# VinAIResearch/GeoFormer

Hardware: AMD Instinct MI355X
Metric: scenes/sec forward (ScanNetV2 ~150k pts) (higher is better)
Workload: dtype f32

## Files before the change

geoformer_amd/_lib.py:

```python
from __future__ import annotations

import ctypes
import os
from ctypes import c_char_p, c_float, c_int, c_longlong, c_size_t, c_uint, c_void_p

from ._build import LIB_PATH

LIB_PATH = os.environ.get("GF_LIB_PATH", LIB_PATH)

_lib = None


class GeoFormerHipError(RuntimeError):
    pass


def _declare(lib):
    P, I, F = c_void_p, c_int, c_float
    sig = {
        "gf_abi_version": (I, []),
        "gf_last_error": (c_char_p, []),
        "gf_index_words": (c_size_t, [I, I, I, I]),
        "gf_index_scratch_bytes": (c_size_t, [c_size_t]),
        "gf_index_build": (I, [P, I, P, I, I, I, I, P, P, P, P, P]),
# ... 15 lines not shown
        "gf_conv_dual_supported": (I, [I, I, I, I, I]),
        "gf_rules_flat_words": (c_size_t, [I, I]),
        "gf_rules_flat_steps": (I, [P, P, I, I, I, I, P, P]),
        "gf_conv_fwd_flat": (I, [P, P, P, P, P, P, I, I, I, I, I, I, P, P, P, P, P, P, P, P]),
        "gf_conv_fwd_dual": (I, [P, P, P, P, P, I, I, I, I, I, I, P, P, P, P, P, P, P, P]),
        "gf_dev_conv_fwd_timed": (I, [P, P, P, P, P, I, I, I, I, I, I, P, P, P, P, P, P, P, P, P]),
        "gf_dev_conv_knobs_g16": (I, [I, I, I, I]),
        "gf_dev_conv_chunks": (I, [I]),
        "gf_dev_conv_g16p_wpb": (I, [I]),
        "gf_dev_conv_knobs": (I, [I, I, I, I, I]),
        "gf_dev_conv_knob_flat": (I, [I, I]),
        "gf_dev_conv_knob_lw": (I, [I, I]),
        "gf_dev_conv_plan": (I, [P, P, P, P, P, P, I, I, I, I, I, I, P, P, P, P, P, P, P, P]),
        "gf_resblock_fwd": (I, [P, P, P, P, P, P, P, I, I, I, I, I, P, P, P, P, P, P, P, P]),
        "gf_conv_wgrad": (I, [P, P, P, I, I, I, I, I, P, P]),
        "gf_conv_wgrad_masked": (I, [P, P, P, P, I, I, I, I, I, P, P]),
        "gf_conv_wgrad_masked_acc": (I, [P, P, P, P, I, I, I, I, I, P, P]),
        "gf_lsap": (I, [P, I, I, P, P, P, P, P, P]),
        "gf_pair_losses_sums_floats": (c_size_t, [I]),
        "gf_pair_losses_fwd": (I, [P, P, P, I, I, I, P, P, P, P]),
        "gf_pair_losses_bwd": (I, [P, P, P, P, I, I, I, P, P, P, P]),
        "gf_unet_ws_bytes": (c_size_t, [P, I, I, I, I, I]),
        "gf_dev_unet_probe": (I, [I]),
        "gf_dev_host_wait_ns": (ctypes.c_ulonglong, [I]),
        "gf_dev_unet_probe_read": (I, [I, P, P]),
        "gf_dev_unet_probe_read2": (I, [I, P, P, P]),
        "gf_dev_conv_kernel_events": (I, [P, P]),
        "gf_dev_conv_kernel_events_taken": (I, []),
        "gf_dev_op_kernel_events": (I, [I, P, P]),
        "gf_dev_op_kernel_events_taken": (I, [I]),
        "gf_dev_event_create": (P, []),
        "gf_dev_event_destroy": (I, [P]),
        "gf_dev_event_elapsed_us": (I, [P, P, P]),
        "gf_unet_fwd": (I, [P, P, P, I, I, I, I, I, P, c_size_t, P, P, P, P]),
        "gf_unet_fwd_phased": (I, [P, P, P, I, I, I, I, I, P, c_size_t, P, P, P, P, P, I, P, P]),
        "gf_unet_fwd_ahead": (I, [P, P, P, I, I, I, I, I, P, c_size_t, P, P, P, P, P, I]),
        "gf_voxelize_fp": (I, [P, P, I, I, I, I, P, P]),
        "gf_voxelize_bp": (I, [P, P, I, I, I, I, P, P]),
        "gf_gather_points": (I, [P, P, I, I, I, I, P, P]),
        "gf_gather_points_grad": (I, [P, P, I, I, I, I, P, P]),
        "gf_group_points": (I, [P, P, I, I, I, I, I, P, P]),
        "gf_group_points_grad": (I, [P, P, I, I, I, I, I, P, P]),
        "gf_ball_query": (I, [P, P, I, I, I, F, I, P, P]),
        "gf_fps_scratch_bytes": (c_size_t, [I]),
        "gf_furthest_point_sampling": (I, [P, I, I, I, P, P, P]),
        "gf_furthest_point_sampling_resume": (I, [P, I, I, I, I, P, P, P]),
        "gf_knn_scratch_bytes": (c_size_t, [I]),
        "gf_knn_radius": (I, [P, I, I, F, I, P, P, P, P, P]),
        "gf_knn_error_flag": (P, [P, I]),
        "gf_geodesic_bfs": (I, [P, P, P, I, I, P, I, F, I, P, P, P, P]),
        "gf_geodesic_bfs_cfg": (I, [P, P, P, I, I, P, I, F, I, P, P, P, c_size_t, I, P]),
        "gf_geodesic_bfs_queue_words": (c_size_t, [I]),
        "gf_dev_cross_attn_bf3": (I, [I]),
        "gf_dev_bfs_qcap_max": (I, [I]),
        "gf_mask_head": (I, [P, P, P, P, P, P, P, P, P, I, I, I, P, P]),
        "gf_mask_head_packed": (I, [P, P, P, P, P, P, P, P, P, I, I, I, I, P, P]),
        "gf_mask_head_episodes": (I, [P, P, P, P, P, P, P, P, P, I, I, I, I, I, P, P, P]),
        "gf_mask_head_split_bytes": (c_size_t, [I]),
        "gf_mask_head_bwd": (I, [P, P, P, P, P, P, P, P, P, I, I, I, I, P, P, P, P]),
        "gf_mask_head_bwd_episodes": (I, [P, P, P, P, P, P, P, P, P, I, I, I, I, I, P, P, P, P]),
        "gf_mask_head_bwd_scratch_floats": (c_size_t, [I, I]),
        "gf_softmax_dim1_fwd": (I, [P, I, I, I, F, P, P]),
        "gf_softmax_dim1_bwd": (I, [P, P, I, I, I, F, P, P]),
        "gf_pointwise_mlp": (I, [P, I, I, P, P, P, P, P, P, P]),
        "gf_pointwise_mlp_rows": (I, [P, P, I, I, P, P, P, P, P, P, P]),
        "gf_group_mlp_max": (I, [P, I, I, I, I, P, P, P, P, P, P, P]),
        "gf_ball_query_centres": (I, [P, P, I, I, I, F, I, P, P, P]),
        "gf_sa_group_mlp_max": (I, [P, P, P, I, I, I, I, F, I, I, I, I, P, P, P, P, P, P, P, P, P, I, P]),
        "gf_ball_query_grid": (I, [P, I, P, P, I, F, I, P, I, P, P, P]),
        "gf_point_grid_build": (I, [P, I, F, P, P]),
        "gf_decoder_token_state_bytes": (c_size_t, [I, I]),
        "gf_decoder_token_stage": (I, [P, P, P, I, I, I, I, I, P, P, P, P, P, P]),
        "gf_mask_intersections_scratch_bytes": (c_size_t, [I, I]),
        "gf_mask_intersections": (I, [P, I, I, P, P, P]),
        "gf_proposal_stats_batched": (I, [P, I, I, P, P, c_longlong, I, F, F, I, I, P, P, P, P, P]),
        "gf_proposal_select_batched": (I, [P, P, P, I, I, P, P, P, P, P]),
        "gf_proposal_scatter_batched": (I, [P, I, I, P, P, I, I, P, F, P, P]),
        "gf_mask_intersections_batched": (I, [P, I, c_longlong, c_longlong, P, P, P]),
        "gf_matrix_nms_batched": (I, [P, I, P, I, F, F, P, P, P]),
        "gf_label_map_batched": (I, [P, I, c_longlong, I, F, P, P, P, P, P, P, P, P, P]),
        "gf_instance_overlaps_scratch_bytes": (c_size_t, [I, I]),
        "gf_instance_overlaps": (I, [P, I, I, P, I, P, P, I, I, P, P, P, P, P, P]),
        "gf_voxelize_idx_scratch_bytes": (c_size_t, [I]),
        "gf_voxelize_idx_count": (I, [P, I, I, I, P, P, P, P]),
        "gf_voxelize_idx_fill": (I, [P, I, I, I, P, P, I, I, P, P, P]),
        "gf_host_legacy_choice": (I, [P, P, c_longlong, c_longlong, P]),
        "gf_host_legacy_prefetch": (I, [P, I, c_longlong]),
        "gf_host_draw_sample": (I, [P, P, c_longlong, c_longlong, P, c_longlong, P, P, P, P, I, P, P, P]),
        "gf_fg_scratch_bytes": (c_size_t, [I]),
        "gf_fg_select": (I, [P, I, I, I, I, P, P, P, P, I, P, P, P, P, P, P, P, P, P]),
        "gf_host_wait_word": (I, [P, I, c_longlong]),
        "gf_proposal_stats": (I, [P, P, P, I, I, I, F, F, I, I, P, P, P, P, P]),
        "gf_proposal_stats_fs": (I, [P, P, I, I, F, F, I, F, P, P, P, P]),
        "gf_proposal_scatter": (I, [P, P, I, I, P, F, I, P, P]),
        "gf_relpos_prepare": (I, [P, P, I, I, I, P, P, P]),
        "gf_proposal_select": (I, [P, P, P, I, P, P, P, P, P]),
        "gf_backbone_transformer_scratch_bytes": (c_size_t, [I]),
        "gf_backbone_transformer_num_params": (I, [I]),
        "gf_backbone_transformer": (I, [P, P, P, I, I, I, I, P, P, P, P]),
        "gf_decoder_pre_train_save_bytes": (c_size_t, [I, I]),
        "gf_decoder_pre_train_work_bytes": (c_size_t, [I, I]),
        "gf_decoder_pre_grad_floats": (c_longlong, []),
        "gf_decoder_pre_train_fwd": (I, [P, P, I, I, P, F, c_uint, I, P, P, P, P]),
        "gf_decoder_pre_train_bwd": (I, [P, P, P, P, P, I, I, P, F, c_uint, I, P, P, P, P, P, P]),
        "gf_decoder_post_train_save_bytes": (c_size_t, [I, I, I]),
        "gf_decoder_post_train_work_bytes": (c_size_t, [I, I, I]),
# ... 150 lines not shown
```

geoformer_amd/csrc/decoder_attn.hip:

```cpp
#include <stdlib.h>

#include "common.h"

#define DA_WAVES 16
#define DA_D 64

__device__ __forceinline__ float da_row_max(float v) {
    v = fmaxf(v, __int_as_float(__builtin_amdgcn_update_dpp(0, __float_as_int(v), 0xB1, 0xF, 0xF, true)));
    v = fmaxf(v, __int_as_float(__builtin_amdgcn_update_dpp(0, __float_as_int(v), 0x4E, 0xF, 0xF, true)));
    v = fmaxf(v, __int_as_float(__builtin_amdgcn_update_dpp(0, __float_as_int(v), 0x141, 0xF, 0xF, true)));
    v = fmaxf(v, __int_as_float(__builtin_amdgcn_update_dpp(0, __float_as_int(v), 0x140, 0xF, 0xF, true)));
    return v;
}
__device__ __forceinline__ float da_row_sum(float v) {
    v += __int_as_float(__builtin_amdgcn_update_dpp(0, __float_as_int(v), 0xB1, 0xF, 0xF, true));
    v += __int_as_float(__builtin_amdgcn_update_dpp(0, __float_as_int(v), 0x4E, 0xF, 0xF, true));
    v += __int_as_float(__builtin_amdgcn_update_dpp(0, __float_as_int(v), 0x141, 0xF, 0xF, true));
    v += __int_as_float(__builtin_amdgcn_update_dpp(0, __float_as_int(v), 0x140, 0xF, 0xF, true));
    return v;
}

template <int WAVES>
__global__ __launch_bounds__(WAVES * 64) void k_decoder_cross_attn(
    const float* __restrict__ geo_ctx, const float* __restrict__ max_geo, const float* __restrict__ qloc,
    const float* __restrict__ cloc, const float* __restrict__ lo, const float* __restrict__ hi,
    const float* __restrict__ gaussB, const float* __restrict__ Q1, const float* __restrict__ K1,
    const float* __restrict__ Kv, const float4* __restrict__ Wpack, int nq, int nc, float* __restrict__ out,
    float* __restrict__ stat_m, float* __restrict__ stat_l) {
    __shared__ float4 sW[3 * 16 * 64];
    __shared__ float4 sQ1[16];
    __shared__ float4 sB[3][2][4];
    __shared__ float sRed[3][WAVES][DA_D];
    const int qi = blockIdx.x, b = blockIdx.y;
    const int tid = threadIdx.x, lane = tid & 63, w = tid >> 6, g = lane >> 4, j = lane & 15;
    for (int t = tid; t < 3 * 16 * 64; t += WAVES * 64) sW[t] = Wpack[t];
    if (tid < 16) sQ1[tid] = *reinterpret_cast<const float4*>(Q1 + ((size_t)b * nq + qi) * DA_D + tid * 4);
    if (tid >= 64 && tid < 64 + 24) {
        const int e = tid - 64, axis = e >> 3, half = (e >> 2) & 1, gg = e & 3;
        sB[axis][half][gg] = *reinterpret_cast<const float4*>(gaussB + axis * 32 + half * 16 + 4 * gg);
    }
    geo_ctx += ((size_t)b * nq + qi) * nc;
    cloc += (size_t)b * nc * 3;
    K1 += (size_t)b * nc * DA_D;
    Kv += (size_t)b * nc * DA_D;
    const float mg = max_geo[(size_t)b * nq + qi];
    const float qx = qloc[((size_t)b * nq + qi) * 3 + 0], qy = qloc[((size_t)b * nq + qi) * 3 + 1],
                qz = qloc[((size_t)b * nq + qi) * 3 + 2];
    const float lx = lo[b * 3 + 0], ly = lo[b * 3 + 1], lz = lo[b * 3 + 2];
    const float sx = hi[b * 3 + 0] - lx, sy = hi[b * 3 + 1] - ly, sz = hi[b * 3 + 2] - lz;
    float sm[4][4], sl[4][4], sa[4][4];
#pragma unroll
    for (int rb = 0; rb < 4; rb++)
#pragma unroll
        for (int r = 0; r < 4; r++) {
            sm[rb][r] = -3.0e38f;
// ... 78 lines not shown
                    const float corr = __expf(sm[rb][r] - mn), p = __expf(x - mn);
                    sl[rb][r] = sl[rb][r] * corr + p;
                    sa[rb][r] = sa[rb][r] * corr + p * val;
                    sm[rb][r] = mn;
                }
            }
            __builtin_amdgcn_sched_barrier(0);
        }
    }
#pragma unroll
    for (int rb = 0; rb < 4; rb++)
#pragma unroll
        for (int r = 0; r < 4; r++) {
            const float m = da_row_max(sm[rb][r]);
            if (j == 0) sRed[0][w][rb * 16 + 4 * g + r] = m;
        }
    __syncthreads();
    if (tid < DA_D) {
        float m = sRed[0][0][tid];
#pragma unroll
        for (int u = 1; u < WAVES; u++) m = fmaxf(m, sRed[0][u][tid]);
        sRed[0][0][tid] = m;
    }
    __syncthreads();
#pragma unroll
    for (int rb = 0; rb < 4; rb++)
#pragma unroll
        for (int r = 0; r < 4; r++) {
            const int c = rb * 16 + 4 * g + r;
            const float f = __expf(sm[rb][r] - sRed[0][0][c]);
            const float l = da_row_sum(sl[rb][r] * f), a = da_row_sum(sa[rb][r] * f);
            if (j == 0) {
                sRed[1][w][c] = l;
                sRed[2][w][c] = a;
            }
        }
    __syncthreads();
    if (tid < DA_D) {
        float L = 0.f, A = 0.f;
#pragma unroll
        for (int u = 0; u < WAVES; u++) {
            L += sRed[1][u][tid];
            A += sRed[2][u][tid];
        }
        out[((size_t)b * nq + qi) * DA_D + tid] = A / L;
        if (stat_m) {
            stat_m[((size_t)b * nq + qi) * DA_D + tid] = sRed[0][0][tid];
            stat_l[((size_t)b * nq + qi) * DA_D + tid] = L;
        }
    }
}

#define DA_WPACK_F32 (3 * 16 * 64 * 4)
#define DA_WPACK_BF3_U4 (3 * 4 * 2 * 3 * 64)
__device__ __forceinline__ void da_split3(float x, unsigned& h, unsigned& m, unsigned& l) {
    h = __float_as_uint(x) & 0xffff0000u;
    const float r1 = x - __uint_as_float(h);
    m = __float_as_uint(r1) & 0xffff0000u;
    l = __float_as_uint(r1 - __uint_as_float(m));
}
typedef __bf16 da_bf16x8 __attribute__((ext_vector_type(8)));
typedef unsigned da_u32x4 __attribute__((ext_vector_type(4)));
struct DaPieces {
    da_u32x4 p[2][3];
};
__device__ __forceinline__ void da_split_pack(const float (&x)[4][4], DaPieces& P) {
#pragma unroll
    for (int h = 0; h < 2; h++) {
        unsigned pc[3][8];
#pragma unroll
        for (int e = 0; e < 8; e++) da_split3(x[2 * h + (e >> 2)][e & 3], pc[0][e], pc[1][e], pc[2][e]);
#pragma unroll
        for (int piece = 0; piece < 3; piece++)
#pragma unroll
            for (int i = 0; i < 4; i++)
                P.p[h][piece][i] = __builtin_amdgcn_perm(pc[piece][2 * i + 1], pc[piece][2 * i], 0x07060302u);
    }
}

#ifndef DA_BF3_WAVES
#define DA_BF3_WAVES 16
#endif
template <int NT>
__device__ __forceinline__ void da_gemm_bf3_n(const uint4* __restrict__ sW3, int m, int rb, int lane, const DaPieces (&X)[NT],
                                              f32x4 (&acc)[NT]) {
#pragma unroll
    for (int h = 0; h < 2; h++) {
        const uint4* w = sW3 + (size_t)(((m * 4 + rb) * 2 + h) * 3) * 64 + lane;
        const da_bf16x8 ah = __builtin_bit_cast(da_bf16x8, w[0]), am = __builtin_bit_cast(da_bf16x8, w[64]),
                        al = __builtin_bit_cast(da_bf16x8, w[128]);
#pragma unroll
        for (int u = 0; u < NT; u++) acc[u] = __builtin_amdgcn_mfma_f32_16x16x32_bf16(al, __builtin_bit_cast(da_bf16x8, X[u].p[h][0]), acc[u], 0, 0, 0);
#pragma unroll
        for (int u = 0; u < NT; u++) acc[u] = __builtin_amdgcn_mfma_f32_16x16x32_bf16(ah, __builtin_bit_cast(da_bf16x8, X[u].p[h][2]), acc[u], 0, 0, 0);
#pragma unroll
        for (int u = 0; u < NT; u++) acc[u] = __builtin_amdgcn_mfma_f32_16x16x32_bf16(am, __builtin_bit_cast(da_bf16x8, X[u].p[h][1]), acc[u], 0, 0, 0);
#pragma unroll
        for (int u = 0; u < NT; u++) acc[u] = __builtin_amdgcn_mfma_f32_16x16x32_bf16(am, __builtin_bit_cast(da_bf16x8, X[u].p[h][0]), acc[u], 0, 0, 0);
#pragma unroll
        for (int u = 0; u < NT; u++) acc[u] = __builtin_amdgcn_mfma_f32_16x16x32_bf16(ah, __builtin_bit_cast(da_bf16x8, X[u].p[h][1]), acc[u], 0, 0, 0);
#pragma unroll
        for (int u = 0; u < NT; u++) acc[u] = __builtin_amdgcn_mfma_f32_16x16x32_bf16(ah, __builtin_bit_cast(da_bf16x8, X[u].p[h][0]), acc[u], 0, 0, 0);
    }
}

template <int WAVES, int NT>
__global__ __launch_bounds__(WAVES * 64) void k_decoder_cross_attn_bf3(
    const float* __restrict__ geo_ctx, const float* __restrict__ max_geo, const float* __restrict__ qloc,
    const float* __restrict__ cloc, const float* __restrict__ lo, const float* __restrict__ hi,
    const float* __restrict__ gaussB, const float* __restrict__ Q1, const float* __restrict__ K1,
    const float* __restrict__ Kv, const uint4* __restrict__ Wp3, int nq, int nc, float* __restrict__ out,
    float* __restrict__ stat_m, float* __restrict__ stat_l) {
    extern __shared__ __attribute__((aligned(16))) unsigned char da_smem[];
    uint4* sW3 = reinterpret_cast<uint4*>(da_smem);
    __shared__ float4 sQ1[16];
    __shared__ float4 sB[3][2][4];
    __shared__ float sRed[3][WAVES][DA_D];
    const int qi = blockIdx.x, b = blockIdx.y;
    const int tid = threadIdx.x, lane = tid & 63, w = tid >> 6, g = lane >> 4, j = lane & 15;
    for (int t = tid; t < DA_WPACK_BF3_U4; t += WAVES * 64) sW3[t] = Wp3[t];
    if (tid < 16) sQ1[tid] = *reinterpret_cast<const float4*>(Q1 + ((size_t)b * nq + qi) * DA_D + tid * 4);
    if (tid >= 64 && tid < 64 + 24) {
        const int e = tid - 64, axis = e >> 3, half = (e >> 2) & 1, gg = e & 3;
        sB[axis][half][gg] = *reinterpret_cast<const float4*>(gaussB + axis * 32 + half * 16 + 4 * gg);
    }
    geo_ctx += ((size_t)b * nq + qi) * nc;
    cloc += (size_t)b * nc * 3;
    K1 += (size_t)b * nc * DA_D;
    Kv += (size_t)b * nc * DA_D;
    const float mg = max_geo[(size_t)b * nq + qi];
    const float qx = qloc[((size_t)b * nq + qi) * 3 + 0], qy = qloc[((size_t)b * nq + qi) * 3 + 1],
                qz = qloc[((size_t)b * nq + qi) * 3 + 2];
    const float lx = lo[b * 3 + 0], ly = lo[b * 3 + 1], lz = lo[b * 3 + 2];
    const float ix = 1.0f / (hi[b * 3 + 0] - lx), iy = 1.0f / (hi[b * 3 + 1] - ly), iz = 1.0f / (hi[b * 3 + 2] - lz);
    constexpr float kScale2 = 0.125f * 1.44269504088896341f;
    float sm[4][4], sl[4][4], sa[4][4];
#pragma unroll
    for (int rb = 0; rb < 4; rb++)
#pragma unroll
        for (int r = 0; r < 4; r++) {
            sm[rb][r] = -3.0e38f;
            sl[rb][r] = 0.f;
            sa[rb][r] = 0.f;
        }
    __syncthreads();

    const int ntiles = (nc + 15) >> 4;
    for (int t0 = w * NT; t0 < ntiles; t0 += WAVES * NT) {
        bool valid[NT];
        int cc[NT];
        DaPieces RP[NT];
#pragma unroll
        for (int u = 0; u < NT; u++) {
            const int ctx = (t0 + u) * 16 + j;
            valid[u] = ctx < nc;
            cc[u] = valid[u] ? ctx : nc - 1;
            const float gd = geo_ctx[cc[u]];
            float g0 = gd, g1 = gd, g2 = gd;
            if (gd < 0.f) {
                g0 = mg + fabsf(qx - cloc[cc[u] * 3 + 0]);
                g1 = mg + fabsf(qy - cloc[cc[u] * 3 + 1]);
                g2 = mg + fabsf(qz - cloc[cc[u] * 3 + 2]);
            }
            const float t0f = (g0 - lx) * ix, t1f = (g1 - ly) * iy, t2f = (g2 - lz) * iz;
            float R[4][4];
#pragma unroll
            for (int half = 0; half < 2; half++) {
                const float4 b0 = sB[0][half][g], b1 = sB[1][half][g], b2v = sB[2][half][g];
                const float p[4] = {fmaf(t2f, b2v.x, fmaf(t1f, b1.x, t0f * b0.x)), fmaf(t2f, b2v.y, fmaf(t1f, b1.y, t0f * b0.y)),
                                    fmaf(t2f, b2v.z, fmaf(t1f, b1.z, t0f * b0.z)), fmaf(t2f, b2v.w, fmaf(t1f, b1.w, t0f * b0.w))};
#pragma unroll
                for (int e = 0; e < 4; e++) {
                    R[half][e] = __builtin_amdgcn_sinf(p[e]);
                    R[2 + half][e] = __builtin_amdgcn_cosf(p[e]);
                }
            }
            da_split_pack(R, RP[u]);
        }
        float H[NT][4][4];
        f32x4 V[NT][4];
#pragma unroll
        for (int rb = 0; rb < 4; rb++) {
            f32x4 acc[NT], vv[NT];
#pragma unroll
            for (int u = 0; u < NT; u++) {
                acc[u] = (f32x4){0.f, 0.f, 0.f, 0.f};
                vv[u] = (f32x4){0.f, 0.f, 0.f, 0.f};
            }
            da_gemm_bf3_n<NT>(sW3, 0, rb, lane, RP, acc);
            const float4 q1 = sQ1[rb * 4 + g];
#pragma unroll
            for (int u = 0; u < NT; u++) {
                const float4 k1 = *reinterpret_cast<const float4*>(K1 + (size_t)cc[u] * DA_D + rb * 16 + 4 * g);
                H[u][rb][0] = fmaxf(acc[u][0] + q1.x - k1.x, 0.f);
                H[u][rb][1] = fmaxf(acc[u][1] + q1.y - k1.y, 0.f);
                H[u][rb][2] = fmaxf(acc[u][2] + q1.z - k1.z, 0.f);
                H[u][rb][3] = fmaxf(acc[u][3] + q1.w - k1.w, 0.f);
            }
            da_gemm_bf3_n<NT>(sW3, 2, rb, lane, RP, vv);
#pragma unroll
            for (int u = 0; u < NT; u++) V[u][rb] = vv[u];
            __builtin_amdgcn_sched_barrier(0);
        }
        DaPieces HP[NT];
#pragma unroll
        for (int u = 0; u < NT; u++) da_split_pack(H[u], HP[u]);
#pragma unroll
        for (int rb = 0; rb < 4; rb++) {
            f32x4 s[NT];
#pragma unroll
            for (int u = 0; u < NT; u++) s[u] = (f32x4){0.f, 0.f, 0.f, 0.f};
            da_gemm_bf3_n<NT>(sW3, 1, rb, lane, HP, s);
#pragma unroll
            for (int u = 0; u < NT; u++) {
                const float4 kv = *reinterpret_cast<const float4*>(Kv + (size_t)cc[u] * DA_D + rb * 16 + 4 * g);
                const float kvv[4] = {kv.x, kv.y, kv.z, kv.w};
                if (valid[u]) {
#pragma unroll
                    for (int r = 0; r < 4; r++) {
                        const float x = s[u][r] * kScale2;
                        const float val = V[u][rb][r] + kvv[r];
                        const float mn = fmaxf(sm[rb][r], x);
                        const float corr = __builtin_amdgcn_exp2f(sm[rb][r] - mn), p = __builtin_amdgcn_exp2f(x - mn);
                        sl[rb][r] = sl[rb][r] * corr + p;
                        sa[rb][r] = sa[rb][r] * corr + p * val;
                        sm[rb][r] = mn;
                    }
                }
            }
            __builtin_amdgcn_sched_barrier(0);
        }
    }
#pragma unroll
    for (int rb = 0; rb < 4; rb++)
#pragma unroll
        for (int r = 0; r < 4; r++) {
            const float m = da_row_max(sm[rb][r]);
            if (j == 0) sRed[0][w][rb * 16 + 4 * g + r] = m;
        }
    __syncthreads();
    if (tid < DA_D) {
        float m = sRed[0][0][tid];
#pragma unroll
        for (int u = 1; u < WAVES; u++) m = fmaxf(m, sRed[0][u][tid]);
        sRed[0][0][tid] = m;
    }
    __syncthreads();
#pragma unroll
    for (int rb = 0; rb < 4; rb++)
#pragma unroll
        for (int r = 0; r < 4; r++) {
            const int c = rb * 16 + 4 * g + r;
            const float f = __builtin_amdgcn_exp2f(sm[rb][r] - sRed[0][0][c]);
            const float l = da_row_sum(sl[rb][r] * f), a = da_row_sum(sa[rb][r] * f);
            if (j == 0) {
                sRed[1][w][c] = l;
                sRed[2][w][c] = a;
            }
        }
    __syncthreads();
    if (tid < DA_D) {
        float L = 0.f, A = 0.f;
#pragma unroll
        for (int u = 0; u < WAVES; u++) {
            L += sRed[1][u][tid];
            A += sRed[2][u][tid];
        }
        out[((size_t)b * nq + qi) * DA_D + tid] = A / L;
        if (stat_m) {
            stat_m[((size_t)b * nq + qi) * DA_D + tid] = sRed[0][0][tid] * 0.69314718055994531f;
            stat_l[((size_t)b * nq + qi) * DA_D + tid] = L;
        }
    }
}

extern "C" size_t gf_decoder_wpack_floats(void) { return (size_t)DA_WPACK_F32 + (size_t)DA_WPACK_BF3_U4 * 4; }

__global__ void k_decoder_pack(const float* __restrict__ W1, const float* __restrict__ W2, const float* __restrict__ Wv,
                               float* __restrict__ Wp) {
    const int t = blockIdx.x * blockDim.x + threadIdx.x;
    if (t >= 3 * 16 * 64 * 4) return;
    const int s = t & 3, lane = (t >> 2) & 63, kb = (t >> 8) & 3, rb = (t >> 10) & 3, m = t >> 12;
    const float* W = m == 0 ? W1 : (m == 1 ? W2 : Wv);
    Wp[t] = W[(rb * 16 + (lane & 15)) * DA_D + kb * 16 + 4 * (lane >> 4) + s];
}

__global__ void k_decoder_pack_bf3(const float* __restrict__ W1, const float* __restrict__ W2, const float* __restrict__ Wv,
                                   uint4* __restrict__ Wp3) {
    const int t = blockIdx.x * blockDim.x + threadIdx.x;
    if (t >= 3 * 4 * 2 * 64) return;
    const int lane = t & 63, h = (t >> 6) & 1, rb = (t >> 7) & 3, m = t >> 9;
    const float* W = m == 0 ? W1 : (m == 1 ? W2 : Wv);
    unsigned pc[3][8];
    for (int e = 0; e < 8; e++) {
        const int kb = 2 * h + (e >> 2), sidx = e & 3;
        da_split3(W[(rb * 16 + (lane & 15)) * DA_D + kb * 16 + 4 * (lane >> 4) + sidx], pc[0][e], pc[1][e], pc[2][e]);
    }
    for (int piece = 0; piece < 3; piece++) {
        uint4 v;
        v.x = (pc[piece][1] & 0xffff0000u) | (pc[piece][0] >> 16);
        v.y = (pc[piece][3] & 0xffff0000u) | (pc[piece][2] >> 16);
        v.z = (pc[piece][5] & 0xffff0000u) | (pc[piece][4] >> 16);
        v.w = (pc[piece][7] & 0xffff0000u) | (pc[piece][6] >> 16);
        Wp3[((size_t)(((m * 4 + rb) * 2 + h) * 3 + piece)) * 64 + lane] = v;
    }
}

extern "C" int gf_decoder_pack_weights(const float* W1, const float* W2, const float* Wv, float* Wpack, void* stream) {
    hipLaunchKernelGGL(k_decoder_pack, dim3(48), dim3(256), 0, (hipStream_t)stream, W1, W2, Wv, Wpack);
    hipLaunchKernelGGL(k_decoder_pack_bf3, dim3(6), dim3(256), 0, (hipStream_t)stream, W1, W2, Wv,
                       reinterpret_cast<uint4*>(Wpack + DA_WPACK_F32));
    GF_CHECK_LAUNCH("gf_decoder_pack_weights");
    return GF_OK;
}

static int g_da_bf3 = -1;
extern "C" int gf_dev_cross_attn_bf3(int on) {
    g_da_bf3 = on < 0 ? -1 : (on != 0);
    return GF_OK;
}

extern "C" int gf_decoder_cross_attn_cfg(const float* geo_ctx, const float* max_geo, const float* qloc, const float* cloc,
                                         const float* lo, const float* hi, const float* gaussB, const float* Q1,
                                         const float* K1, const float* Kv, const float* Wpack, const float* b2, int B,
                                         int nq, int nc, int d, float* out, float* stat_m, float* stat_l, int wg_waves,
                                         void* stream) {
    GF_CHECK_ARG(d == DA_D, "gf_decoder_cross_attn: implemented for dec_dim = 64 (got %d)", d);
    GF_CHECK_ARG(B >= 0 && nq >= 0 && nc >= 1, "gf_decoder_cross_attn: bad sizes");
    GF_CHECK_ARG((stat_m == nullptr) == (stat_l == nullptr), "gf_decoder_cross_attn: stat_m and stat_l come together");
    GF_CHECK_ARG(wg_waves == 16 || wg_waves == 8, "gf_decoder_cross_attn_cfg: %d waves per workgroup (16 or 8)", wg_waves);
    if (B == 0 || nq == 0) return GF_OK;
    (void)b2;
    if (wg_waves == 16 && g_da_bf3 != 0) {
        const size_t lds = (size_t)DA_WPACK_BF3_U4 * sizeof(uint4);
        gf_allow_lds((const void*)k_decoder_cross_attn_bf3<DA_BF3_WAVES, 1>, (int)lds);
        GF_LAUNCH_OP(GF_OP_CROSS_ATTN, (k_decoder_cross_attn_bf3<DA_BF3_WAVES, 1>), dim3(nq, B), dim3(DA_BF3_WAVES * 64), lds,
                     (hipStream_t)stream, geo_ctx, max_geo, qloc, cloc, lo, hi, gaussB, Q1, K1, Kv,
                     reinterpret_cast<const uint4*>(Wpack + DA_WPACK_F32), nq, nc, out, stat_m, stat_l);
        GF_CHECK_LAUNCH("gf_decoder_cross_attn");
        return GF_OK;
    }
    if (wg_waves == 16)
        GF_LAUNCH_OP(GF_OP_CROSS_ATTN, k_decoder_cross_attn<16>, dim3(nq, B), dim3(16 * 64), 0, (hipStream_t)stream, geo_ctx,
                     max_geo, qloc, cloc, lo, hi, gaussB, Q1, K1, Kv, reinterpret_cast<const float4*>(Wpack), nq, nc, out,
                     stat_m, stat_l);
    else
        GF_LAUNCH_OP(GF_OP_CROSS_ATTN, k_decoder_cross_attn<8>, dim3(nq, B), dim3(8 * 64), 0, (hipStream_t)stream, geo_ctx,
                     max_geo, qloc, cloc, lo, hi, gaussB, Q1, K1, Kv, reinterpret_cast<const float4*>(Wpack), nq, nc, out,
                     stat_m, stat_l);
    GF_CHECK_LAUNCH("gf_decoder_cross_attn");
    return GF_OK;
}

extern "C" int gf_decoder_cross_attn(const float* geo_ctx, const float* max_geo, const float* qloc, const float* cloc,
                                     const float* lo, const float* hi, const float* gaussB, const float* Q1,
                                     const float* K1, const float* Kv, const float* Wpack, const float* b2, int B,
                                     int nq, int nc, int d, float* out, float* stat_m, float* stat_l, void* stream) {
    return gf_decoder_cross_attn_cfg(geo_ctx, max_geo, qloc, cloc, lo, hi, gaussB, Q1, K1, Kv, Wpack, b2, B, nq, nc, d, out,
                                     stat_m, stat_l, 16, stream);
}


#define DAB_TS 68

__global__ void k_decoder_pack_w2t(const float* __restrict__ W2, float* __restrict__ Wp) {
    const int t = blockIdx.x * blockDim.x + threadIdx.x;
    if (t >= 16 * 64 * 4) return;
    const int s = t & 3, lane = (t >> 2) & 63, kb = (t >> 8) & 3, cb = (t >> 10) & 3;
    Wp[t] = W2[(kb * 16 + 4 * (lane >> 4) + s) * DA_D + cb * 16 + (lane & 15)];
}

__global__ __launch_bounds__(256, 1) void k_decoder_cross_attn_bwd(
    const float* __restrict__ geo_ctx, const float* __restrict__ max_geo, const float* __restrict__ qloc,
    const float* __restrict__ cloc, const float* __restrict__ lo, const float* __restrict__ hi,
    const float* __restrict__ gaussB, const float* __restrict__ Q1, const float* __restrict__ K1,
    const float* __restrict__ Kv, const float4* __restrict__ Wpack, const float4* __restrict__ W2Tpack,
    const float* __restrict__ outv, const float* __restrict__ stat_m, const float* __restrict__ stat_l,
    const float* __restrict__ gout, int B, int nq, int nc, int qsplit, float* __restrict__ dQ1p,
    float* __restrict__ dK1, float* __restrict__ dKv, float* __restrict__ dWp) {
    __shared__ float4 sW[3 * 16 * 64];
    __shared__ float4 sW2T[16 * 64];
    __shared__ float4 sB[3][2][4];
    __shared__ __attribute__((aligned(16))) float sT[4][16 * DAB_TS];
    __shared__ __attribute__((aligned(16))) float sV[4][4][DA_D];
    const int tid = threadIdx.x, lane = tid & 63, w = tid >> 6, g = lane >> 4, j = lane & 15;
    for (int t = tid; t < 3 * 16 * 64; t += 256) sW[t] = Wpack[t];
    for (int t = tid; t < 16 * 64; t += 256) sW2T[t] = W2Tpack[t];
    if (tid < 24) {
        const int axis = tid >> 3, half = (tid >> 2) & 1, gg = tid & 3;
        sB[axis][half][gg] = *reinterpret_cast<const float4*>(gaussB + axis * 32 + half * 16 + 4 * gg);
    }
// ... 290 lines not shown
```

geoformer_amd/csrc/tile_gemm.h:

```cpp
#pragma once
#include "common.h"

__device__ __forceinline__ f32x4 gf_mfma4(float4 a, float4 b, f32x4 acc) {
    acc = __builtin_amdgcn_mfma_f32_16x16x4f32(a.x, b.x, acc, 0, 0, 0);
    acc = __builtin_amdgcn_mfma_f32_16x16x4f32(a.y, b.y, acc, 0, 0, 0);
    acc = __builtin_amdgcn_mfma_f32_16x16x4f32(a.z, b.z, acc, 0, 0, 0);
    acc = __builtin_amdgcn_mfma_f32_16x16x4f32(a.w, b.w, acc, 0, 0, 0);
    return acc;
}

template <bool RELU, typename Epi>
__device__ __forceinline__ void gf_tile_gemm(const float* A, int lda, int nvalid, int K, const float* __restrict__ W,
                                             const float* __restrict__ bias, int N, int wave, int nwaves, int lane,
                                             Epi epi, const float* __restrict__ addend = nullptr, int add_ld = 0) {
    const int j = lane & 15, g = lane >> 4;
    const int KC = K >> 4;
    for (int ct = wave; ct < (N >> 4); ct += nwaves) {
        const float* xa = A + (size_t)j * lda + 4 * g;
        const float* wb = W + (size_t)(ct * 16 + j) * K + 4 * g;
        const int col = ct * 16 + j;
        const float bs = bias[col];
        float ad[4] = {0.f, 0.f, 0.f, 0.f};
        if (addend) {
#pragma unroll
// ... 46 lines not shown
    const int j = lane & 15, g = lane >> 4;
    const float* xa = A + (size_t)j * lda + 4 * g;
#pragma unroll
    for (int t = 0; t < NT; t++) {
        const int ct = wave + t * nwaves;
        if (ct >= (N >> 4)) break;
        const int col = ct * 16 + j;
        float ad[4] = {0.f, 0.f, 0.f, 0.f};
        if (addend) {
#pragma unroll
            for (int i = 0; i < 4; i++)
                if (4 * g + i < nvalid) ad[i] = addend[(size_t)(4 * g + i) * add_ld + col];
        }
        f32x4 acc = {0.f, 0.f, 0.f, 0.f};
#pragma unroll
        for (int kc = 0; kc < KC; kc++) {
            if (kc < (K >> 4)) {
                float4 a = j < nvalid ? *reinterpret_cast<const float4*>(xa + kc * 16) : make_float4(0.f, 0.f, 0.f, 0.f);
                acc = gf_mfma4(a, w.b[t][kc], acc);
            }
        }
#pragma unroll
        for (int i = 0; i < 4; i++) {
            const int r = 4 * g + i;
            if (r >= nvalid) continue;
            float v = acc[i] + w.bias[t];
            if (RELU) v = fmaxf(v, 0.f);
            if (addend) v += ad[i];
            epi(r, col, v);
        }
    }
}

template <typename Epi>
__device__ __forceinline__ void gf_tile_gemm_t(const float* A, int lda, int K, const float* __restrict__ W, int ldw, int N,
                                               int wave, int nwaves, int lane, Epi epi) {
    const int j = lane & 15, g = lane >> 4;
    const int KC = K >> 4;
    for (int ct = wave; ct < (N >> 4); ct += nwaves) {
        const float* xa = A + (size_t)j * lda + 4 * g;
        const float* wb = W + (size_t)(4 * g) * ldw + ct * 16 + j;
        f32x4 acc = {0.f, 0.f, 0.f, 0.f};
#pragma unroll 2
        for (int kc = 0; kc < KC; kc++) {
            const float4 a = *reinterpret_cast<const float4*>(xa + kc * 16);
            const float* w = wb + (size_t)kc * 16 * ldw;
            const float4 b = make_float4(w[0], w[ldw], w[2 * (size_t)ldw], w[3 * (size_t)ldw]);
            acc = gf_mfma4(a, b, acc);
        }
#pragma unroll
        for (int i = 0; i < 4; i++) epi(4 * g + i, ct * 16 + j, acc[i]);
    }
}
```

include/geoformer_hip_dev.h:

```cpp
#ifndef GEOFORMER_HIP_DEV_H
#define GEOFORMER_HIP_DEV_H

#include "geoformer_hip.h"

#ifdef __cplusplus
extern "C" {
#endif

int gf_dev_conv_fwd_timed(const float* in, const float* Wp, const int32_t* nbr, const uint32_t* gmask,
                          const int32_t* steps, int K, int M_in, int M_out, int ld, int Cin, int Cout, const float* in_scale, const float* in_shift,
                          const float* residual, const float* out_scale, const float* out_shift, float* out, void* ev_start,
                          void* ev_stop, void* stream);

int gf_dev_conv_knobs(int split, int wide, int pair, int ldsw, int block);

int gf_dev_conv_knobs_g16(int use, int ldsw, int gpw, int pipe);

int gf_dev_conv_knob_flat(int use, int max_items);

int gf_dev_conv_knob_lw(int use, int min_groups);

int gf_dev_conv_plan(const float* in, const float* Wp, const int32_t* nbr, const uint32_t* gmask, const int32_t* steps,
                     const int32_t* flat, int K, int M_in, int M_out, int ld, int Cin, int Cout, const float* in_scale,
                     const float* in_shift, const float* residual, const float* out_scale, const float* out_shift, float* out,
                     float* out_act, int* desc);

int gf_dev_conv_chunks(int n);
int gf_dev_conv_g16p_wpb(int wpb);

int gf_dev_unet_probe(int mode);
unsigned long long gf_dev_host_wait_ns(int reset);
int gf_dev_unet_probe_read(int max_records, int* meta, float* us);
int gf_dev_unet_probe_read2(int max_records, int* meta, float* us, float* us_kernel);
int gf_dev_conv_kernel_events(void* start, void* stop);
int gf_dev_conv_kernel_events_taken(void);

int gf_dev_op_kernel_events(int op, void* start, void* stop);
int gf_dev_op_kernel_events_taken(int op);
void* gf_dev_event_create(void);
int gf_dev_event_destroy(void* event);
int gf_dev_event_elapsed_us(void* start, void* stop, float* us);

int gf_dev_cross_attn_bf3(int on);

int gf_dev_bfs_qcap_max(int qcap);

#ifdef __cplusplus
}
#endif
#endif
```

Baseline: 229.7.

## Replace bf16x3 split GEMMs in decoder cross-attention with scaled f16x2 split

The decoder cross-attention kernel emulated fp32 matmuls with a three-piece bf16 split that needed six MFMAs per k-chunk. It now uses a two-piece f16 split with power-of-two scaling (per-matrix for weights, per-tile for the hidden activations), which needs three MFMAs per chunk and less packing work and LDS. The online softmax also gains a default single-exp update that derives corr and p from one exp2 of -|delta|, with the old two-exp form kept behind a toggle. The NT multi-tile template is dropped, and debug helpers for the f16 split and MFMA are added. The risk is reduced accuracy or overflow at the f16 range edges, since the result relies on the scaling to stay close to fp32.

```diff
diff --git a/geoformer_amd/_lib.py b/geoformer_amd/_lib.py
--- a/geoformer_amd/_lib.py
+++ b/geoformer_amd/_lib.py
@@ -91,6 +91,9 @@
         "gf_geodesic_bfs_cfg": (I, [P, P, P, I, I, P, I, F, I, P, P, P, c_size_t, I, P]),
         "gf_geodesic_bfs_queue_words": (c_size_t, [I]),
         "gf_dev_cross_attn_bf3": (I, [I]),
+        "gf_dev_cross_attn_two_exp": (I, [I]),
+        "gf_dev_f16_split": (I, [P, P, I, P, P, P, P, P]),
+        "gf_dev_mfma_f16": (I, [P, P, I, P, P]),
         "gf_dev_bfs_qcap_max": (I, [I]),
         "gf_mask_head": (I, [P, P, P, P, P, P, P, P, P, I, I, I, P, P]),
         "gf_mask_head_packed": (I, [P, P, P, P, P, P, P, P, P, I, I, I, I, P, P]),
diff --git a/geoformer_amd/csrc/decoder_attn.hip b/geoformer_amd/csrc/decoder_attn.hip
--- a/geoformer_amd/csrc/decoder_attn.hip
+++ b/geoformer_amd/csrc/decoder_attn.hip
@@ -1,6 +1,7 @@
 #include <stdlib.h>
 
 #include "common.h"
+#include "tile_gemm.h"
 
 #define DA_WAVES 16
 #define DA_D 64
@@ -185,73 +186,56 @@
 }
 
 #define DA_WPACK_F32 (3 * 16 * 64 * 4)
-#define DA_WPACK_BF3_U4 (3 * 4 * 2 * 3 * 64)
-__device__ __forceinline__ void da_split3(float x, unsigned& h, unsigned& m, unsigned& l) {
-    h = __float_as_uint(x) & 0xffff0000u;
-    const float r1 = x - __uint_as_float(h);
-    m = __float_as_uint(r1) & 0xffff0000u;
-    l = __float_as_uint(r1 - __uint_as_float(m));
-}
-typedef __bf16 da_bf16x8 __attribute__((ext_vector_type(8)));
+#define DA_WPACK_F16_U4 (3 * 4 * 2 * 2 * 64)
+#define DA_R_SCALE 8192.0f
 typedef unsigned da_u32x4 __attribute__((ext_vector_type(4)));
 struct DaPieces {
-    da_u32x4 p[2][3];
+    da_u32x4 p[2][2];
 };
-__device__ __forceinline__ void da_split_pack(const float (&x)[4][4], DaPieces& P) {
+__device__ __forceinline__ void da_split_pack(const float (&x)[4][4], float scale, DaPieces& P) {
+#pragma unroll
+    for (int h = 0; h < 2; h++)
+#pragma unroll
+        for (int i = 0; i < 4; i++) {
+            unsigned ph, pm;
+            gf_f16_split2(x[2 * h + (i >> 1)][2 * (i & 1)], x[2 * h + (i >> 1)][2 * (i & 1) + 1], scale, ph, pm);
+            P.p[h][0][i] = ph;
+            P.p[h][1][i] = pm;
+        }
+}
+
+#ifndef DA_F16_WAVES
+#define DA_F16_WAVES 16
+#endif
+__device__ __forceinline__ void da_gemm_f16(const uint4* __restrict__ sW2, int m, int rb, int lane, const DaPieces& X, f32x4& acc) {
 #pragma unroll
     for (int h = 0; h < 2; h++) {
-        unsigned pc[3][8];
-#pragma unroll
-        for (int e = 0; e < 8; e++) da_split3(x[2 * h + (e >> 2)][e & 3], pc[0][e], pc[1][e], pc[2][e]);
-#pragma unroll
-        for (int piece = 0; piece < 3; piece++)
-#pragma unroll
-            for (int i = 0; i < 4; i++)
-                P.p[h][piece][i] = __builtin_amdgcn_perm(pc[piece][2 * i + 1], pc[piece][2 * i], 0x07060302u);
-    }
-}
-
-#ifndef DA_BF3_WAVES
-#define DA_BF3_WAVES 16
-#endif
-template <int NT>
-__device__ __forceinline__ void da_gemm_bf3_n(const uint4* __restrict__ sW3, int m, int rb, int lane, const DaPieces (&X)[NT],
-                                              f32x4 (&acc)[NT]) {
-#pragma unroll
-    for (int h = 0; h < 2; h++) {
-        const uint4* w = sW3 + (size_t)(((m * 4 + rb) * 2 + h) * 3) * 64 + lane;
-        const da_bf16x8 ah = __builtin_bit_cast(da_bf16x8, w[0]), am = __builtin_bit_cast(da_bf16x8, w[64]),
-                        al = __builtin_bit_cast(da_bf16x8, w[128]);
-#pragma unroll
-        for (int u = 0; u < NT; u++) acc[u] = __builtin_amdgcn_mfma_f32_16x16x32_bf16(al, __builtin_bit_cast(da_bf16x8, X[u].p[h][0]), acc[u], 0, 0, 0);
-#pragma unroll
-        for (int u = 0; u < NT; u++) acc[u] = __builtin_amdgcn_mfma_f32_16x16x32_bf16(ah, __builtin_bit_cast(da_bf16x8, X[u].p[h][2]), acc[u], 0, 0, 0);
-#pragma unroll
-        for (int u = 0; u < NT; u++) acc[u] = __builtin_amdgcn_mfma_f32_16x16x32_bf16(am, __builtin_bit_cast(da_bf16x8, X[u].p[h][1]), acc[u], 0, 0, 0);
-#pragma unroll
-        for (int u = 0; u < NT; u++) acc[u] = __builtin_amdgcn_mfma_f32_16x16x32_bf16(am, __builtin_bit_cast(da_bf16x8, X[u].p[h][0]), acc[u], 0, 0, 0);
-#pragma unroll
-        for (int u = 0; u < NT; u++) acc[u] = __builtin_amdgcn_mfma_f32_16x16x32_bf16(ah, __builtin_bit_cast(da_bf16x8, X[u].p[h][1]), acc[u], 0, 0, 0);
-#pragma unroll
-        for (int u = 0; u < NT; u++) acc[u] = __builtin_amdgcn_mfma_f32_16x16x32_bf16(ah, __builtin_bit_cast(da_bf16x8, X[u].p[h][0]), acc[u], 0, 0, 0);
-    }
-}
-
-template <int WAVES, int NT>
-__global__ __launch_bounds__(WAVES * 64) void k_decoder_cross_attn_bf3(
+        const uint4* w = sW2 + (size_t)(((m * 4 + rb) * 2 + h) * 2) * 64 + lane;
+        const gf_f16x8 ah = __builtin_bit_cast(gf_f16x8, w[0]), am = __builtin_bit_cast(gf_f16x8, w[64]);
+        const gf_f16x8 xh = __builtin_bit_cast(gf_f16x8, X.p[h][0]), xm = __builtin_bit_cast(gf_f16x8, X.p[h][1]);
+        acc = __builtin_amdgcn_mfma_f32_16x16x32_f16(am, xh, acc, 0, 0, 0);
+        acc = __builtin_amdgcn_mfma_f32_16x16x32_f16(ah, xm, acc, 0, 0, 0);
+        acc = __builtin_amdgcn_mfma_f32_16x16x32_f16(ah, xh, acc, 0, 0, 0);
+    }
+}
+
+template <int WAVES, bool TWO_EXP>
+__global__ __launch_bounds__(WAVES * 64) void k_decoder_cross_attn_f16(
     const float* __restrict__ geo_ctx, const float* __restrict__ max_geo, const float* __restrict__ qloc,
     const float* __restrict__ cloc, const float* __restrict__ lo, const float* __restrict__ hi,
     const float* __restrict__ gaussB, const float* __restrict__ Q1, const float* __restrict__ K1,
-    const float* __restrict__ Kv, const uint4* __restrict__ Wp3, int nq, int nc, float* __restrict__ out,
+    const float* __restrict__ Kv, const uint4* __restrict__ Wp2, int nq, int nc, float* __restrict__ out,
     float* __restrict__ stat_m, float* __restrict__ stat_l) {
     extern __shared__ __attribute__((aligned(16))) unsigned char da_smem[];
-    uint4* sW3 = reinterpret_cast<uint4*>(da_smem);
+    uint4* sW2 = reinterpret_cast<uint4*>(da_smem);
     __shared__ float4 sQ1[16];
     __shared__ float4 sB[3][2][4];
     __shared__ float sRed[3][WAVES][DA_D];
     const int qi = blockIdx.x, b = blockIdx.y;
     const int tid = threadIdx.x, lane = tid & 63, w = tid >> 6, g = lane >> 4, j = lane & 15;
-    for (int t = tid; t < DA_WPACK_BF3_U4; t += WAVES * 64) sW3[t] = Wp3[t];
+    for (int t = tid; t < DA_WPACK_F16_U4; t += WAVES * 64) sW2[t] = Wp2[t];
+    const float* wsc = reinterpret_cast<const float*>(Wp2 + DA_WPACK_F16_U4);
+    const float inv1 = wsc[0], inv2 = wsc[1], invv = wsc[2];
     if (tid < 16) sQ1[tid] = *reinterpret_cast<const float4*>(Q1 + ((size_t)b * nq + qi) * DA_D + tid * 4);
     if (tid >= 64 && tid < 64 + 24) {
         const int e = tid - 64, axis = e >> 3, half = (e >> 2) & 1, gg = e & 3;
@@ -267,6 +251,7 @@
     const float lx = lo[b * 3 + 0], ly = lo[b * 3 + 1], lz = lo[b * 3 + 2];
     const float ix = 1.0f / (hi[b * 3 + 0] - lx), iy = 1.0f / (hi[b * 3 + 1] - ly), iz = 1.0f / (hi[b * 3 + 2] - lz);
     constexpr float kScale2 = 0.125f * 1.44269504088896341f;
+    const float kScale2W = kScale2 * inv2;
     float sm[4][4], sl[4][4], sa[4][4];
 #pragma unroll
     for (int rb = 0; rb < 4; rb++)
@@ -279,21 +264,18 @@
     __syncthreads();
 
     const int ntiles = (nc + 15) >> 4;
-    for (int t0 = w * NT; t0 < ntiles; t0 += WAVES * NT) {
-        bool valid[NT];
-        int cc[NT];
-        DaPieces RP[NT];
-#pragma unroll
-        for (int u = 0; u < NT; u++) {
-            const int ctx = (t0 + u) * 16 + j;
-            valid[u] = ctx < nc;
-            cc[u] = valid[u] ? ctx : nc - 1;
-            const float gd = geo_ctx[cc[u]];
+    for (int t0 = w; t0 < ntiles; t0 += WAVES) {
+        const int ctx = t0 * 16 + j;
+        const bool valid = ctx < nc;
+        const int cc = valid ? ctx : nc - 1;
+        DaPieces RP;
+        {
+            const float gd = geo_ctx[cc];
             float g0 = gd, g1 = gd, g2 = gd;
             if (gd < 0.f) {
-                g0 = mg + fabsf(qx - cloc[cc[u] * 3 + 0]);
-                g1 = mg + fabsf(qy - cloc[cc[u] * 3 + 1]);
-                g2 = mg + fabsf(qz - cloc[cc[u] * 3 + 2]);
+                g0 = mg + fabsf(qx - cloc[cc * 3 + 0]);
+                g1 = mg + fabsf(qy - cloc[cc * 3 + 1]);
+                g2 = mg + fabsf(qz - cloc[cc * 3 + 2]);
             }
             const float t0f = (g0 - lx) * ix, t1f = (g1 - ly) * iy, t2f = (g2 - lz) * iz;
             float R[4][4];
@@ -308,57 +290,61 @@
                     R[2 + half][e] = __builtin_amdgcn_cosf(p[e]);
                 }
             }
-            da_split_pack(R, RP[u]);
-        }
-        float H[NT][4][4];
-        f32x4 V[NT][4];
+            da_split_pack(R, DA_R_SCALE, RP);
+        }
+        float H[4][4];
+        f32x4 V[4];
 #pragma unroll
         for (int rb = 0; rb < 4; rb++) {
-            f32x4 acc[NT], vv[NT];
-#pragma unroll
-            for (int u = 0; u < NT; u++) {
-                acc[u] = (f32x4){0.f, 0.f, 0.f, 0.f};
-                vv[u] = (f32x4){0.f, 0.f, 0.f, 0.f};
-            }
-            da_gemm_bf3_n<NT>(sW3, 0, rb, lane, RP, acc);
+            f32x4 acc = (f32x4){0.f, 0.f, 0.f, 0.f}, vv = (f32x4){0.f, 0.f, 0.f, 0.f};
+            da_gemm_f16(sW2, 0, rb, lane, RP, acc);
             const float4 q1 = sQ1[rb * 4 + g];
-#pragma unroll
-            for (int u = 0; u < NT; u++) {
-                const float4 k1 = *reinterpret_cast<const float4*>(K1 + (size_t)cc[u] * DA_D + rb * 16 + 4 * g);
-                H[u][rb][0] = fmaxf(acc[u][0] + q1.x - k1.x, 0.f);
-                H[u][rb][1] = fmaxf(acc[u][1] + q1.y - k1.y, 0.f);
-                H[u][rb][2] = fmaxf(acc[u][2] + q1.z - k1.z, 0.f);
-                H[u][rb][3] = fmaxf(acc[u][3] + q1.w - k1.w, 0.f);
-            }
-            da_gemm_bf3_n<NT>(sW3, 2, rb, lane, RP, vv);
-#pragma unroll
-            for (int u = 0; u < NT; u++) V[u][rb] = vv[u];
+            const float4 k1 = *reinterpret_cast<const float4*>(K1 + (size_t)cc * DA_D + rb * 16 + 4 * g);
+            H[rb][0] = fmaxf(fmaf(acc[0], inv1, q1.x) - k1.x, 0.f);
+            H[rb][1] = fmaxf(fmaf(acc[1], inv1, q1.y) - k1.y, 0.f);
+            H[rb][2] = fmaxf(fmaf(acc[2], inv1, q1.z) - k1.z, 0.f);
+            H[rb][3] = fmaxf(fmaf(acc[3], inv1, q1.w) - k1.w, 0.f);
+            da_gemm_f16(sW2, 2, rb, lane, RP, vv);
+            V[rb] = vv;
             __builtin_amdgcn_sched_barrier(0);
         }
-        DaPieces HP[NT];
-#pragma unroll
-        for (int u = 0; u < NT; u++) da_split_pack(H[u], HP[u]);
+        int hb = 0;
+#pragma unroll
+        for (int rb = 0; rb < 4; rb++)
+#pragma unroll
+            for (int r = 0; r < 4; r++) hb = max(hb, __float_as_int(H[rb][r]));
+        hb = max(hb, gf_shfl_xor_i<16>(hb));
+        hb = max(hb, gf_shfl_xor_i<32>(hb));
+        float hs, hinv;
+        gf_f16_scale(__int_as_float(hb), hs, hinv);
+        const float xs = kScale2W * hinv;
+        DaPieces HP;
+        da_split_pack(H, hs, HP);
 #pragma unroll
         for (int rb = 0; rb < 4; rb++) {
-            f32x4 s[NT];
-#pragma unroll
-            for (int u = 0; u < NT; u++) s[u] = (f32x4){0.f, 0.f, 0.f, 0.f};
-            da_gemm_bf3_n<NT>(sW3, 1, rb, lane, HP, s);
-#pragma unroll
-            for (int u = 0; u < NT; u++) {
-                const float4 kv = *reinterpret_cast<const float4*>(Kv + (size_t)cc[u] * DA_D + rb * 16 + 4 * g);
-                const float kvv[4] = {kv.x, kv.y, kv.z, kv.w};
-                if (valid[u]) {
-#pragma unroll
-                    for (int r = 0; r < 4; r++) {
-                        const float x = s[u][r] * kScale2;
-                        const float val = V[u][rb][r] + kvv[r];
-                        const float mn = fmaxf(sm[rb][r], x);
-                        const float corr = __builtin_amdgcn_exp2f(sm[rb][r] - mn), p = __builtin_amdgcn_exp2f(x - mn);
-                        sl[rb][r] = sl[rb][r] * corr + p;
-                        sa[rb][r] = sa[rb][r] * corr + p * val;
-                        sm[rb][r] = mn;
+            f32x4 s = (f32x4){0.f, 0.f, 0.f, 0.f};
+            da_gemm_f16(sW2, 1, rb, lane, HP, s);
+            const float4 kv = *reinterpret_cast<const float4*>(Kv + (size_t)cc * DA_D + rb * 16 + 4 * g);
+            const float kvv[4] = {kv.x, kv.y, kv.z, kv.w};
+            if (valid) {
+#pragma unroll
+                for (int r = 0; r < 4; r++) {
+                    const float x = s[r] * xs;
+                    const float val = fmaf(V[rb][r], invv, kvv[r]);
+                    const float mn = fmaxf(sm[rb][r], x);
+                    float corr, p;
+                    if constexpr (TWO_EXP) {
+                        corr = __builtin_amdgcn_exp2f(sm[rb][r] - mn);
+                        p = __builtin_amdgcn_exp2f(x - mn);
+                    } else {
+                        const float dlt = x - sm[rb][r];
+                        const float e = __builtin_amdgcn_exp2f(-fabsf(dlt));
+                        corr = dlt > 0.f ? e : 1.f;
+                        p = dlt > 0.f ? 1.f : e;
                     }
+                    sl[rb][r] = sl[rb][r] * corr + p;
+                    sa[rb][r] = sa[rb][r] * corr + p * val;
+                    sm[rb][r] = mn;
                 }
             }
             __builtin_amdgcn_sched_barrier(0);
@@ -407,7 +393,7 @@
     }
 }
 
-extern "C" size_t gf_decoder_wpack_floats(void) { return (size_t)DA_WPACK_F32 + (size_t)DA_WPACK_BF3_U4 * 4; }
+extern "C" size_t gf_decoder_wpack_floats(void) { return (size_t)DA_WPACK_F32 + (size_t)DA_WPACK_F16_U4 * 4 + 4; }
 
 __global__ void k_decoder_pack(const float* __restrict__ W1, const float* __restrict__ W2, const float* __restrict__ Wv,
                                float* __restrict__ Wp) {
@@ -418,30 +404,35 @@
     Wp[t] = W[(rb * 16 + (lane & 15)) * DA_D + kb * 16 + 4 * (lane >> 4) + s];
 }
 
-__global__ void k_decoder_pack_bf3(const float* __restrict__ W1, const float* __restrict__ W2, const float* __restrict__ Wv,
-                                   uint4* __restrict__ Wp3) {
-    const int t = blockIdx.x * blockDim.x + threadIdx.x;
-    if (t >= 3 * 4 * 2 * 64) return;
-    const int lane = t & 63, h = (t >> 6) & 1, rb = (t >> 7) & 3, m = t >> 9;
+__global__ __launch_bounds__(256) void k_decoder_pack_f16(const float* __restrict__ W1, const float* __restrict__ W2,
+                                                          const float* __restrict__ Wv, uint4* __restrict__ Wp2) {
+    __shared__ float red[256];
+    const int t = threadIdx.x, m = blockIdx.x;
     const float* W = m == 0 ? W1 : (m == 1 ? W2 : Wv);
-    unsigned pc[3][8];
-    for (int e = 0; e < 8; e++) {
-        const int kb = 2 * h + (e >> 2), sidx = e & 3;
-        da_split3(W[(rb * 16 + (lane & 15)) * DA_D + kb * 16 + 4 * (lane >> 4) + sidx], pc[0][e], pc[1][e], pc[2][e]);
-    }
-    for (int piece = 0; piece < 3; piece++) {
-        uint4 v;
-        v.x = (pc[piece][1] & 0xffff0000u) | (pc[piece][0] >> 16);
-        v.y = (pc[piece][3] & 0xffff0000u) | (pc[piece][2] >> 16);
-        v.z = (pc[piece][5] & 0xffff0000u) | (pc[piece][4] >> 16);
-        v.w = (pc[piece][7] & 0xffff0000u) | (pc[piece][6] >> 16);
-        Wp3[((size_t)(((m * 4 + rb) * 2 + h) * 3 + piece)) * 64 + lane] = v;
-    }
+    float a = 0.f;
+    for (int i = 0; i < 16; i++) a = fmaxf(a, fabsf(W[t * 16 + i]));
+    red[t] = a;
+    __syncthreads();
+    for (int i = 0; i < 256; i++) a = fmaxf(a, red[i]);
+    float scale, inv;
+    gf_f16_scale(a, scale, inv);
+    for (int u = t; u < 4 * 2 * 64; u += 256) {
+        const int lane = u & 63, h = (u >> 6) & 1, rb = u >> 7;
+        unsigned ph[4], pm[4];
+        for (int i = 0; i < 4; i++) {
+            const float* src = W + (rb * 16 + (lane & 15)) * DA_D + (2 * h + (i >> 1)) * 16 + 4 * (lane >> 4) + 2 * (i & 1);
+            gf_f16_split2(src[0], src[1], scale, ph[i], pm[i]);
+        }
+        Wp2[((size_t)(((m * 4 + rb) * 2 + h) * 2 + 0)) * 64 + lane] = make_uint4(ph[0], ph[1], ph[2], ph[3]);
+        Wp2[((size_t)(((m * 4 + rb) * 2 + h) * 2 + 1)) * 64 + lane] = make_uint4(pm[0], pm[1], pm[2], pm[3]);
+    }
+    if (t == 0) reinterpret_cast<float*>(Wp2 + DA_WPACK_F16_U4)[m] = m == 1 ? inv : inv * (1.0f / DA_R_SCALE);
+    if (t == 1 && m == 0) reinterpret_cast<float*>(Wp2 + DA_WPACK_F16_U4)[3] = 0.f;
 }
 
 extern "C" int gf_decoder_pack_weights(const float* W1, const float* W2, const float* Wv, float* Wpack, void* stream) {
     hipLaunchKernelGGL(k_decoder_pack, dim3(48), dim3(256), 0, (hipStream_t)stream, W1, W2, Wv, Wpack);
-    hipLaunchKernelGGL(k_decoder_pack_bf3, dim3(6), dim3(256), 0, (hipStream_t)stream, W1, W2, Wv,
+    hipLaunchKernelGGL(k_decoder_pack_f16, dim3(3), dim3(256), 0, (hipStream_t)stream, W1, W2, Wv,
                        reinterpret_cast<uint4*>(Wpack + DA_WPACK_F32));
     GF_CHECK_LAUNCH("gf_decoder_pack_weights");
     return GF_OK;
@@ -450,6 +441,11 @@
 static int g_da_bf3 = -1;
 extern "C" int gf_dev_cross_attn_bf3(int on) {
     g_da_bf3 = on < 0 ? -1 : (on != 0);
+    return GF_OK;
+}
+static int g_da_two_exp = 0;
+extern "C" int gf_dev_cross_attn_two_exp(int on) {
+    g_da_two_exp = on > 0;
     return GF_OK;
 }
 
@@ -465,11 +461,19 @@
     if (B == 0 || nq == 0) return GF_OK;
     (void)b2;
     if (wg_waves == 16 && g_da_bf3 != 0) {
-        const size_t lds = (size_t)DA_WPACK_BF3_U4 * sizeof(uint4);
-        gf_allow_lds((const void*)k_decoder_cross_attn_bf3<DA_BF3_WAVES, 1>, (int)lds);
-        GF_LAUNCH_OP(GF_OP_CROSS_ATTN, (k_decoder_cross_attn_bf3<DA_BF3_WAVES, 1>), dim3(nq, B), dim3(DA_BF3_WAVES * 64), lds,
-                     (hipStream_t)stream, geo_ctx, max_geo, qloc, cloc, lo, hi, gaussB, Q1, K1, Kv,
-                     reinterpret_cast<const uint4*>(Wpack + DA_WPACK_F32), nq, nc, out, stat_m, stat_l);
+        const size_t lds = (size_t)DA_WPACK_F16_U4 * sizeof(uint4);
+        const uint4* wp2 = reinterpret_cast<const uint4*>(Wpack + DA_WPACK_F32);
+        if (g_da_two_exp) {
+            gf_allow_lds((const void*)k_decoder_cross_attn_f16<DA_F16_WAVES, true>, (int)lds);
+            GF_LAUNCH_OP(GF_OP_CROSS_ATTN, (k_decoder_cross_attn_f16<DA_F16_WAVES, true>), dim3(nq, B), dim3(DA_F16_WAVES * 64), lds,
+                         (hipStream_t)stream, geo_ctx, max_geo, qloc, cloc, lo, hi, gaussB, Q1, K1, Kv, wp2, nq, nc, out, stat_m,
+                         stat_l);
+        } else {
+            gf_allow_lds((const void*)k_decoder_cross_attn_f16<DA_F16_WAVES, false>, (int)lds);
+            GF_LAUNCH_OP(GF_OP_CROSS_ATTN, (k_decoder_cross_attn_f16<DA_F16_WAVES, false>), dim3(nq, B), dim3(DA_F16_WAVES * 64), lds,
+                         (hipStream_t)stream, geo_ctx, max_geo, qloc, cloc, lo, hi, gaussB, Q1, K1, Kv, wp2, nq, nc, out, stat_m,
+                         stat_l);
+        }
         GF_CHECK_LAUNCH("gf_decoder_cross_attn");
         return GF_OK;
     }
diff --git a/geoformer_amd/csrc/f16_split_dev.hip b/geoformer_amd/csrc/f16_split_dev.hip
--- /dev/null
+++ b/geoformer_amd/csrc/f16_split_dev.hip
@@ -0,0 +1,63 @@
+#include "common.h"
+#include "tile_gemm.h"
+
+__global__ void k_dev_f16_split(const float* __restrict__ x, const float* __restrict__ amax, int n, unsigned short* __restrict__ h,
+                                unsigned short* __restrict__ m, float* __restrict__ scale, float* __restrict__ inv) {
+    const int i = blockIdx.x * blockDim.x + threadIdx.x;
+    if (i >= n) return;
+    float s, si;
+    gf_f16_scale(amax[i], s, si);
+    unsigned ph, pm;
+    gf_f16_split2(x[i], 0.f, s, ph, pm);
+    h[i] = (unsigned short)(ph & 0xffffu);
+    m[i] = (unsigned short)(pm & 0xffffu);
+    scale[i] = s;
+    inv[i] = si;
+}
+
+typedef _Float16 dev_f16x4 __attribute__((ext_vector_type(4)));
+template <int K>
+__global__ __launch_bounds__(64) void k_dev_mfma_f16(const float* __restrict__ A, const float* __restrict__ B, float* __restrict__ D) {
+    constexpr int KL = K / 4;
+    const int lane = threadIdx.x, g = lane >> 4, j = lane & 15;
+    f32x4 acc = {0.f, 0.f, 0.f, 0.f};
+    if constexpr (K == 32) {
+        gf_f16x8 a, b;
+#pragma unroll
+        for (int e = 0; e < KL; e++) {
+            a[e] = (_Float16)A[j * K + KL * g + e];
+            b[e] = (_Float16)B[(KL * g + e) * 16 + j];
+        }
+        acc = __builtin_amdgcn_mfma_f32_16x16x32_f16(a, b, acc, 0, 0, 0);
+    } else {
+        dev_f16x4 a, b;
+#pragma unroll
+        for (int e = 0; e < KL; e++) {
+            a[e] = (_Float16)A[j * K + KL * g + e];
+            b[e] = (_Float16)B[(KL * g + e) * 16 + j];
+        }
+        acc = __builtin_amdgcn_mfma_f32_16x16x16f16(a, b, acc, 0, 0, 0);
+    }
+#pragma unroll
+    for (int r = 0; r < 4; r++) D[(4 * g + r) * 16 + j] = acc[r];
+}
+
+extern "C" int gf_dev_f16_split(const float* x, const float* amax, int n, void* h, void* m, float* scale, float* inv,
+                                void* stream) {
+    GF_CHECK_ARG(n >= 0, "gf_dev_f16_split: bad size");
+    if (n == 0) return GF_OK;
+    hipLaunchKernelGGL(k_dev_f16_split, dim3(gf_div_up(n, 256)), dim3(256), 0, (hipStream_t)stream, x, amax, n,
+                       (unsigned short*)h, (unsigned short*)m, scale, inv);
+    GF_CHECK_LAUNCH("gf_dev_f16_split");
+    return GF_OK;
+}
+
+extern "C" int gf_dev_mfma_f16(const float* A, const float* B, int K, float* D, void* stream) {
+    GF_CHECK_ARG(K == 32 || K == 16, "gf_dev_mfma_f16: K = 32 or 16 (got %d)", K);
+    if (K == 32)
+        hipLaunchKernelGGL(k_dev_mfma_f16<32>, dim3(1), dim3(64), 0, (hipStream_t)stream, A, B, D);
+    else
+        hipLaunchKernelGGL(k_dev_mfma_f16<16>, dim3(1), dim3(64), 0, (hipStream_t)stream, A, B, D);
+    GF_CHECK_LAUNCH("gf_dev_mfma_f16");
+    return GF_OK;
+}
diff --git a/geoformer_amd/csrc/tile_gemm.h b/geoformer_amd/csrc/tile_gemm.h
--- a/geoformer_amd/csrc/tile_gemm.h
+++ b/geoformer_amd/csrc/tile_gemm.h
@@ -122,3 +122,18 @@
         for (int i = 0; i < 4; i++) epi(4 * g + i, ct * 16 + j, acc[i]);
     }
 }
+
+typedef _Float16 gf_f16x8 __attribute__((ext_vector_type(8)));
+typedef _Float16 gf_f16x2 __attribute__((ext_vector_type(2)));
+
+__device__ __forceinline__ void gf_f16_scale(float amax, float& scale, float& inv) {
+    const int eb = max((int)((__float_as_uint(amax) >> 23) & 0xffu), 14);
+    scale = __uint_as_float((unsigned)(267 - eb) << 23);
+    inv = __uint_as_float((unsigned)(eb - 13) << 23);
+}
+__device__ __forceinline__ void gf_f16_split2(float x0, float x1, float scale, unsigned& h, unsigned& m) {
+    const gf_f16x2 hh = {(_Float16)(x0 * scale), (_Float16)(x1 * scale)};
+    const gf_f16x2 mm = {(_Float16)fmaf(x0, scale, -(float)hh[0]), (_Float16)fmaf(x1, scale, -(float)hh[1])};
+    h = __builtin_bit_cast(unsigned, hh);
+    m = __builtin_bit_cast(unsigned, mm);
+}
diff --git a/include/geoformer_hip_dev.h b/include/geoformer_hip_dev.h
--- a/include/geoformer_hip_dev.h
+++ b/include/geoformer_hip_dev.h
@@ -42,6 +42,10 @@
 int gf_dev_event_elapsed_us(void* start, void* stop, float* us);
 
 int gf_dev_cross_attn_bf3(int on);
+int gf_dev_cross_attn_two_exp(int on);
+
+int gf_dev_f16_split(const float* x, const float* amax, int n, void* h, void* m, float* scale, float* inv, void* stream);
+int gf_dev_mfma_f16(const float* A, const float* B, int K, float* D, void* stream);
 
 int gf_dev_bfs_qcap_max(int qcap);
 
```

New measurement: 229.6, median of 2. About the same (-0.0%).
